# ZHKKKe/PixelSSL

Measured on NVIDIA H100. Metric: images/sec DeepLab-v2-R101 MT 513x513 bs16, higher is better.
Workload: dtype f16x3 (fp16 pairs, fp32 accumulate)

## Files before the change

### pixelssl_b200/csrc/conv_tc.cu

```cuda
#include "common.cuh"
#include <cuda.h>
#include <cstdlib>

typedef CUresult (*EncodeTiledFn)(CUtensorMap*, CUtensorMapDataType, cuuint32_t, void*, const cuuint64_t*,
                                  const cuuint64_t*, const cuuint32_t*, const cuuint32_t*, CUtensorMapInterleave,
                                  CUtensorMapSwizzle, CUtensorMapL2promotion, CUtensorMapFloatOOBfill);
static EncodeTiledFn get_encode() {
    static EncodeTiledFn fn = nullptr;
    if (!fn) {
        void* p = nullptr;
        cudaDriverEntryPointQueryResult q;
        if (cudaGetDriverEntryPoint("cuTensorMapEncodeTiled", &p, cudaEnableDefault, &q) == cudaSuccess &&
            q == cudaDriverEntryPointSuccess)
            fn = (EncodeTiledFn)p;
    }
    return fn;
}

static int make_act_map(CUtensorMap* m, const void* base, int C, int W, int H, int N, int bw, int bh, int estride = 1, int f16 = 0) {
    EncodeTiledFn enc = get_encode();
    if (!enc) return PXL_ERR_UNSUPPORTED;
    const cuuint64_t eb = f16 ? 2 : 4;
    cuuint64_t dims[4] = {(cuuint64_t)C, (cuuint64_t)W, (cuuint64_t)H, (cuuint64_t)N};
    cuuint64_t strides[3] = {(cuuint64_t)C * eb, (cuuint64_t)W * C * eb, (cuuint64_t)H * W * C * eb};
    cuuint32_t box[4] = {(cuuint32_t)(f16 ? 64 : 32), (cuuint32_t)(bw * estride), (cuuint32_t)(bh * estride), 1};
    cuuint32_t es[4] = {1, (cuuint32_t)estride, (cuuint32_t)estride, 1};
    if (box[1] > 256 || box[2] > 256) return PXL_ERR_UNSUPPORTED;
    CUresult r = enc(m, f16 ? CU_TENSOR_MAP_DATA_TYPE_FLOAT16 : CU_TENSOR_MAP_DATA_TYPE_FLOAT32, 4, (void*)base, dims, strides, box, es,
                     CU_TENSOR_MAP_INTERLEAVE_NONE, CU_TENSOR_MAP_SWIZZLE_128B, CU_TENSOR_MAP_L2_PROMOTION_L2_256B,
                     CU_TENSOR_MAP_FLOAT_OOB_FILL_NONE);
    return r == CUDA_SUCCESS ? 0 : PXL_ERR_BAD_ARG;
}

static int make_w_map(CUtensorMap* m, const void* base, int64_t K, int rows, int bn, int f16 = 0) {
    EncodeTiledFn enc = get_encode();
    if (!enc) return PXL_ERR_UNSUPPORTED;
    cuuint64_t dims[2] = {(cuuint64_t)K, (cuuint64_t)rows};
    cuuint64_t strides[1] = {(cuuint64_t)K * (f16 ? 2 : 4)};
    cuuint32_t box[2] = {(cuuint32_t)(f16 ? 64 : 32), (cuuint32_t)bn};
    cuuint32_t es[2] = {1, 1};
    CUresult r = enc(m, f16 ? CU_TENSOR_MAP_DATA_TYPE_FLOAT16 : CU_TENSOR_MAP_DATA_TYPE_FLOAT32, 2, (void*)base, dims, strides, box, es,
                     CU_TENSOR_MAP_INTERLEAVE_NONE, CU_TENSOR_MAP_SWIZZLE_128B, CU_TENSOR_MAP_L2_PROMOTION_L2_256B,
                     CU_TENSOR_MAP_FLOAT_OOB_FILL_NONE);
    return r == CUDA_SUCCESS ? 0 : PXL_ERR_BAD_ARG;
}

__device__ __forceinline__ uint32_t smem_u32(const void* p) { return (uint32_t)__cvta_generic_to_shared(p); }

__device__ __forceinline__ void mbar_init(uint64_t* bar, uint32_t count) {
    asm volatile("mbarrier.init.shared::cta.b64 [%0], %1;" ::"r"(smem_u32(bar)), "r"(count));
}
__device__ __forceinline__ void mbar_expect_tx(uint64_t* bar, uint32_t bytes) {
    asm volatile("mbarrier.arrive.expect_tx.shared::cta.b64 _, [%0], %1;" ::"r"(smem_u32(bar)), "r"(bytes) : "memory");
}
__device__ __forceinline__ void mbar_arrive(uint64_t* bar) {
    asm volatile("mbarrier.arrive.shared::cta.b64 _, [%0];" ::"r"(smem_u32(bar)) : "memory");
}
__device__ __forceinline__ bool mbar_try_wait(uint64_t* bar, uint32_t parity) {
    uint32_t ok;
    asm volatile(
        "{\n\t.reg .pred p;\n\t"
        "mbarrier.try_wait.parity.shared::cta.b64 p, [%1], %2;\n\t"
        "selp.u32 %0, 1, 0, p;\n\t}"
        : "=r"(ok)
        : "r"(smem_u32(bar)), "r"(parity)
        : "memory");
    return ok != 0;
}
__device__ __forceinline__ bool mbar_wait(uint64_t* bar, uint32_t parity, int* flag, int code) {
    for (uint32_t spin = 0; spin < (1u << 22); ++spin) {
        if (mbar_try_wait(bar, parity)) return true;
        if ((spin & 1023u) == 1023u && *(volatile int*)flag != 0) return false;
    }
    atomicCAS(flag, 0, code);
    return false;
}
__device__ __forceinline__ void tma_load_4d(void* dst, const CUtensorMap* map, uint64_t* bar, int c0, int c1, int c2, int c3) {
    asm volatile(
        "cp.async.bulk.tensor.4d.shared::cluster.global.mbarrier::complete_tx::bytes [%0], [%1, {%3, %4, %5, %6}], [%2];"
        ::"r"(smem_u32(dst)), "l"(map), "r"(smem_u32(bar)), "r"(c0), "r"(c1), "r"(c2), "r"(c3)
        : "memory");
}
__device__ __forceinline__ void tma_load_2d(void* dst, const CUtensorMap* map, uint64_t* bar, int c0, int c1) {
    asm volatile(
        "cp.async.bulk.tensor.2d.shared::cluster.global.mbarrier::complete_tx::bytes [%0], [%1, {%3, %4}], [%2];"
        ::"r"(smem_u32(dst)), "l"(map), "r"(smem_u32(bar)), "r"(c0), "r"(c1)
        : "memory");
}
__device__ __forceinline__ bool elect_one() {
    uint32_t pred = 0;
    asm volatile(
        "{\n\t.reg .b32 rx;\n\t.reg .pred px;\n\t"
        "elect.sync rx|px, 0xffffffff;\n\t"
        "@px mov.s32 %0, 1;\n\t}"
        : "+r"(pred));
    return pred != 0;
}
__device__ __forceinline__ void named_bar(int id, int count) {
    asm volatile("bar.sync %0, %1;" ::"r"(id), "r"(count) : "memory");
}
__device__ __forceinline__ void fence_async_smem() { asm volatile("fence.proxy.async.shared::cta;" ::: "memory"); }

__device__ __forceinline__ uint64_t sw128_desc(uint32_t smem_addr, uint32_t lbo_bytes = 16) {
    uint64_t d = 0;
    d |= (uint64_t)((smem_addr & 0x3FFFF) >> 4);
    d |= (uint64_t)((lbo_bytes >> 4) & 0x3FFF) << 16;
    d |= (uint64_t)(1024 >> 4) << 32;
    d |= (uint64_t)1 << 62;
    return d;
}
__device__ __forceinline__ void wg_arrive() { asm volatile("wgmma.fence.sync.aligned;" ::: "memory"); }
__device__ __forceinline__ void wg_commit() { asm volatile("wgmma.commit_group.sync.aligned;" ::: "memory"); }
__device__ __forceinline__ void wg_wait0() { asm volatile("wgmma.wait_group.sync.aligned 0;" ::: "memory"); }
template <int R>
__device__ __forceinline__ void fence_regs(float (&d)[R]) {
#pragma unroll
    for (int i = 0; i < R; ++i) asm volatile("" : "+f"(d[i])::"memory");
}

template <int N, int KIND>
__device__ __forceinline__ void wgmma_op(float (&d)[N / 2], uint64_t da, uint64_t db, int scale_d);
template <> __device__ __forceinline__ void wgmma_op<32, 0>(float (&d)[16], uint64_t da, uint64_t db, int scale_d) {
    asm volatile(
        "{\n\t.reg .pred p;\n\tsetp.ne.b32 p, %18, 0;\n\t"
        "wgmma.mma_async.sync.aligned.m64n32k8.f32.tf32.tf32 {%0, %1, %2, %3, %4, %5, %6, %7, %8, %9, %10, %11, %12, %13, %14, %15}, %16, %17, p, 1, 1;\n\t}"
        : "+f"(d[0]), "+f"(d[1]), "+f"(d[2]), "+f"(d[3]), "+f"(d[4]), "+f"(d[5]), "+f"(d[6]), "+f"(d[7]), "+f"(d[8]), "+f"(d[9]), "+f"(d[10]), "+f"(d[11]), "+f"(d[12]), "+f"(d[13]), "+f"(d[14]), "+f"(d[15])
        : "l"(da), "l"(db), "r"(scale_d));
}
template <> __device__ __forceinline__ void wgmma_op<64, 0>(float (&d)[32], uint64_t da, uint64_t db, int scale_d) {
    asm volatile(
        "{\n\t.reg .pred p;\n\tsetp.ne.b32 p, %34, 0;\n\t"
        "wgmma.mma_async.sync.aligned.m64n64k8.f32.tf32.tf32 {%0, %1, %2, %3, %4, %5, %6, %7, %8, %9, %10, %11, %12, %13, %14, %15, %16, %17, %18, %19, %20, %21, %22, %23, %24, %25, %26, %27, %28, %29, %30, %31}, %32, %33, p, 1, 1;\n\t}"
        : "+f"(d[0]), "+f"(d[1]), "+f"(d[2]), "+f"(d[3]), "+f"(d[4]), "+f"(d[5]), "+f"(d[6]), "+f"(d[7]), "+f"(d[8]), "+f"(d[9]), "+f"(d[10]), "+f"(d[11]), "+f"(d[12]), "+f"(d[13]), "+f"(d[14]), "+f"(d[15]), "+f"(d[16]), "+f"(d[17]), "+f"(d[18]), "+f"(d[19]), "+f"(d[20]), "+f"(d[21]), "+f"(d[22]), "+f"(d[23]), "+f"(d[24]), "+f"(d[25]), "+f"(d[26]), "+f"(d[27]), "+f"(d[28]), "+f"(d[29]), "+f"(d[30]), "+f"(d[31])
        : "l"(da), "l"(db), "r"(scale_d));
}
template <> __device__ __forceinline__ void wgmma_op<128, 0>(float (&d)[64], uint64_t da, uint64_t db, int scale_d) {
    asm volatile(
        "{\n\t.reg .pred p;\n\tsetp.ne.b32 p, %66, 0;\n\t"
        "wgmma.mma_async.sync.aligned.m64n128k8.f32.tf32.tf32 {%0, %1, %2, %3, %4, %5, %6, %7, %8, %9, %10, %11, %12, %13, %14, %15, %16, %17, %18, %19, %20, %21, %22, %23, %24, %25, %26, %27, %28, %29, %30, %31, %32, %33, %34, %35, %36, %37, %38, %39, %40, %41, %42, %43, %44, %45, %46, %47, %48, %49, %50, %51, %52, %53, %54, %55, %56, %57, %58, %59, %60, %61, %62, %63}, %64, %65, p, 1, 1;\n\t}"
        : "+f"(d[0]), "+f"(d[1]), "+f"(d[2]), "+f"(d[3]), "+f"(d[4]), "+f"(d[5]), "+f"(d[6]), "+f"(d[7]), "+f"(d[8]), "+f"(d[9]), "+f"(d[10]), "+f"(d[11]), "+f"(d[12]), "+f"(d[13]), "+f"(d[14]), "+f"(d[15]), "+f"(d[16]), "+f"(d[17]), "+f"(d[18]), "+f"(d[19]), "+f"(d[20]), "+f"(d[21]), "+f"(d[22]), "+f"(d[23]), "+f"(d[24]), "+f"(d[25]), "+f"(d[26]), "+f"(d[27]), "+f"(d[28]), "+f"(d[29]), "+f"(d[30]), "+f"(d[31]), "+f"(d[32]), "+f"(d[33]), "+f"(d[34]), "+f"(d[35]), "+f"(d[36]), "+f"(d[37]), "+f"(d[38]), "+f"(d[39]), "+f"(d[40]), "+f"(d[41]), "+f"(d[42]), "+f"(d[43]), "+f"(d[44]), "+f"(d[45]), "+f"(d[46]), "+f"(d[47]), "+f"(d[48]), "+f"(d[49]), "+f"(d[50]), "+f"(d[51]), "+f"(d[52]), "+f"(d[53]), "+f"(d[54]), "+f"(d[55]), "+f"(d[56]), "+f"(d[57]), "+f"(d[58]), "+f"(d[59]), "+f"(d[60]), "+f"(d[61]), "+f"(d[62]), "+f"(d[63])
        : "l"(da), "l"(db), "r"(scale_d));
}
template <> __device__ __forceinline__ void wgmma_op<32, 1>(float (&d)[16], uint64_t da, uint64_t db, int scale_d) {
    asm volatile(
        "{\n\t.reg .pred p;\n\tsetp.ne.b32 p, %18, 0;\n\t"
        "wgmma.mma_async.sync.aligned.m64n32k16.f32.f16.f16 {%0, %1, %2, %3, %4, %5, %6, %7, %8, %9, %10, %11, %12, %13, %14, %15}, %16, %17, p, 1, 1, 0, 0;\n\t}"
        : "+f"(d[0]), "+f"(d[1]), "+f"(d[2]), "+f"(d[3]), "+f"(d[4]), "+f"(d[5]), "+f"(d[6]), "+f"(d[7]), "+f"(d[8]), "+f"(d[9]), "+f"(d[10]), "+f"(d[11]), "+f"(d[12]), "+f"(d[13]), "+f"(d[14]), "+f"(d[15])
        : "l"(da), "l"(db), "r"(scale_d));
}
template <> __device__ __forceinline__ void wgmma_op<64, 1>(float (&d)[32], uint64_t da, uint64_t db, int scale_d) {
    asm volatile(
        "{\n\t.reg .pred p;\n\tsetp.ne.b32 p, %34, 0;\n\t"
        "wgmma.mma_async.sync.aligned.m64n64k16.f32.f16.f16 {%0, %1, %2, %3, %4, %5, %6, %7, %8, %9, %10, %11, %12, %13, %14, %15, %16, %17, %18, %19, %20, %21, %22, %23, %24, %25, %26, %27, %28, %29, %30, %31}, %32, %33, p, 1, 1, 0, 0;\n\t}"
        : "+f"(d[0]), "+f"(d[1]), "+f"(d[2]), "+f"(d[3]), "+f"(d[4]), "+f"(d[5]), "+f"(d[6]), "+f"(d[7]), "+f"(d[8]), "+f"(d[9]), "+f"(d[10]), "+f"(d[11]), "+f"(d[12]), "+f"(d[13]), "+f"(d[14]), "+f"(d[15]), "+f"(d[16]), "+f"(d[17]), "+f"(d[18]), "+f"(d[19]), "+f"(d[20]), "+f"(d[21]), "+f"(d[22]), "+f"(d[23]), "+f"(d[24]), "+f"(d[25]), "+f"(d[26]), "+f"(d[27]), "+f"(d[28]), "+f"(d[29]), "+f"(d[30]), "+f"(d[31])
        : "l"(da), "l"(db), "r"(scale_d));
}
template <> __device__ __forceinline__ void wgmma_op<128, 1>(float (&d)[64], uint64_t da, uint64_t db, int scale_d) {
    asm volatile(
        "{\n\t.reg .pred p;\n\tsetp.ne.b32 p, %66, 0;\n\t"
        "wgmma.mma_async.sync.aligned.m64n128k16.f32.f16.f16 {%0, %1, %2, %3, %4, %5, %6, %7, %8, %9, %10, %11, %12, %13, %14, %15, %16, %17, %18, %19, %20, %21, %22, %23, %24, %25, %26, %27, %28, %29, %30, %31, %32, %33, %34, %35, %36, %37, %38, %39, %40, %41, %42, %43, %44, %45, %46, %47, %48, %49, %50, %51, %52, %53, %54, %55, %56, %57, %58, %59, %60, %61, %62, %63}, %64, %65, p, 1, 1, 0, 0;\n\t}"
        : "+f"(d[0]), "+f"(d[1]), "+f"(d[2]), "+f"(d[3]), "+f"(d[4]), "+f"(d[5]), "+f"(d[6]), "+f"(d[7]), "+f"(d[8]), "+f"(d[9]), "+f"(d[10]), "+f"(d[11]), "+f"(d[12]), "+f"(d[13]), "+f"(d[14]), "+f"(d[15]), "+f"(d[16]), "+f"(d[17]), "+f"(d[18]), "+f"(d[19]), "+f"(d[20]), "+f"(d[21]), "+f"(d[22]), "+f"(d[23]), "+f"(d[24]), "+f"(d[25]), "+f"(d[26]), "+f"(d[27]), "+f"(d[28]), "+f"(d[29]), "+f"(d[30]), "+f"(d[31]), "+f"(d[32]), "+f"(d[33]), "+f"(d[34]), "+f"(d[35]), "+f"(d[36]), "+f"(d[37]), "+f"(d[38]), "+f"(d[39]), "+f"(d[40]), "+f"(d[41]), "+f"(d[42]), "+f"(d[43]), "+f"(d[44]), "+f"(d[45]), "+f"(d[46]), "+f"(d[47]), "+f"(d[48]), "+f"(d[49]), "+f"(d[50]), "+f"(d[51]), "+f"(d[52]), "+f"(d[53]), "+f"(d[54]), "+f"(d[55]), "+f"(d[56]), "+f"(d[57]), "+f"(d[58]), "+f"(d[59]), "+f"(d[60]), "+f"(d[61]), "+f"(d[62]), "+f"(d[63])
        : "l"(da), "l"(db), "r"(scale_d));
}
template <> __device__ __forceinline__ void wgmma_op<64, 2>(float (&d)[32], uint64_t da, uint64_t db, int scale_d) {
    asm volatile(
        "{\n\t.reg .pred p;\n\tsetp.ne.b32 p, %34, 0;\n\t"
        "wgmma.mma_async.sync.aligned.m64n64k16.f32.f16.f16 {%0, %1, %2, %3, %4, %5, %6, %7, %8, %9, %10, %11, %12, %13, %14, %15, %16, %17, %18, %19, %20, %21, %22, %23, %24, %25, %26, %27, %28, %29, %30, %31}, %32, %33, p, 1, 1, 1, 1;\n\t}"
        : "+f"(d[0]), "+f"(d[1]), "+f"(d[2]), "+f"(d[3]), "+f"(d[4]), "+f"(d[5]), "+f"(d[6]), "+f"(d[7]), "+f"(d[8]), "+f"(d[9]), "+f"(d[10]), "+f"(d[11]), "+f"(d[12]), "+f"(d[13]), "+f"(d[14]), "+f"(d[15]), "+f"(d[16]), "+f"(d[17]), "+f"(d[18]), "+f"(d[19]), "+f"(d[20]), "+f"(d[21]), "+f"(d[22]), "+f"(d[23]), "+f"(d[24]), "+f"(d[25]), "+f"(d[26]), "+f"(d[27]), "+f"(d[28]), "+f"(d[29]), "+f"(d[30]), "+f"(d[31])
        : "l"(da), "l"(db), "r"(scale_d));
}
template <> __device__ __forceinline__ void wgmma_op<128, 2>(float (&d)[64], uint64_t da, uint64_t db, int scale_d) {
    asm volatile(
        "{\n\t.reg .pred p;\n\tsetp.ne.b32 p, %66, 0;\n\t"
        "wgmma.mma_async.sync.aligned.m64n128k16.f32.f16.f16 {%0, %1, %2, %3, %4, %5, %6, %7, %8, %9, %10, %11, %12, %13, %14, %15, %16, %17, %18, %19, %20, %21, %22, %23, %24, %25, %26, %27, %28, %29, %30, %31, %32, %33, %34, %35, %36, %37, %38, %39, %40, %41, %42, %43, %44, %45, %46, %47, %48, %49, %50, %51, %52, %53, %54, %55, %56, %57, %58, %59, %60, %61, %62, %63}, %64, %65, p, 1, 1, 1, 1;\n\t}"
        : "+f"(d[0]), "+f"(d[1]), "+f"(d[2]), "+f"(d[3]), "+f"(d[4]), "+f"(d[5]), "+f"(d[6]), "+f"(d[7]), "+f"(d[8]), "+f"(d[9]), "+f"(d[10]), "+f"(d[11]), "+f"(d[12]), "+f"(d[13]), "+f"(d[14]), "+f"(d[15]), "+f"(d[16]), "+f"(d[17]), "+f"(d[18]), "+f"(d[19]), "+f"(d[20]), "+f"(d[21]), "+f"(d[22]), "+f"(d[23]), "+f"(d[24]), "+f"(d[25]), "+f"(d[26]), "+f"(d[27]), "+f"(d[28]), "+f"(d[29]), "+f"(d[30]), "+f"(d[31]), "+f"(d[32]), "+f"(d[33]), "+f"(d[34]), "+f"(d[35]), "+f"(d[36]), "+f"(d[37]), "+f"(d[38]), "+f"(d[39]), "+f"(d[40]), "+f"(d[41]), "+f"(d[42]), "+f"(d[43]), "+f"(d[44]), "+f"(d[45]), "+f"(d[46]), "+f"(d[47]), "+f"(d[48]), "+f"(d[49]), "+f"(d[50]), "+f"(d[51]), "+f"(d[52]), "+f"(d[53]), "+f"(d[54]), "+f"(d[55]), "+f"(d[56]), "+f"(d[57]), "+f"(d[58]), "+f"(d[59]), "+f"(d[60]), "+f"(d[61]), "+f"(d[62]), "+f"(d[63])
        : "l"(da), "l"(db), "r"(scale_d));
}

template <int BN, int F16>
__device__ __forceinline__ void mma_slice(float (&part)[BN / 2], float (&corr)[BN / 2], uint64_t da, uint64_t db, uint64_t dal,
                                          uint64_t dbl, bool split3) {
#pragma unroll
    for (int k = 0; k < 4; ++k) wgmma_op<BN, F16>(part, da + 2 * k, db + 2 * k, k);
    if (split3) {
#pragma unroll
        for (int k = 0; k < 4; ++k) wgmma_op<BN, F16>(corr, dal + 2 * k, db + 2 * k, k);
#pragma unroll
        for (int k = 0; k < 4; ++k) wgmma_op<BN, F16>(corr, da + 2 * k, dbl + 2 * k, 1);
    }
}

__device__ __forceinline__ float4 tf32_split4(float4 v, float4& lo) {
    float4 h;
    const float* vp = &v.x; float* hp = &h.x; float* lp = &lo.x;
#pragma unroll
    for (int e = 0; e < 4; ++e) {
        uint32_t u;
        asm("cvt.rna.tf32.f32 %0, %1;" : "=r"(u) : "f"(vp[e]));
        u &= 0xFFFFE000u;
        hp[e] = __uint_as_float(u);
        lp[e] = vp[e] - hp[e];
    }
    return h;
}

struct TcParams {
    int Cin, Cout, ldo, ntaps, kchunks;
    int N, OH, OW;
    int BW, BH, tilesW, tilesH;
    int stages, nsplit;
    int a_inkernel;
    int in_mul;
    int out_mul, out_offy, out_offx, outH, outW;
    int ntilesN, pix_tiles, total_tiles;
    int kc;
    float out_scale;
    int out_acc;
    short dy[PXL_MAX_TAPS], dx[PXL_MAX_TAPS], widx[PXL_MAX_TAPS];
};

#define TC_A_BYTES (128 * 128)
#define TC_MAX_STAGES 8
#define TC_THREADS 384

__device__ __forceinline__ void tc_tile_coords(const TcParams& p, int tile, int bn, int& n0, int& w0, int& h0, int& n) {
    const int nt = tile / p.pix_tiles, pix = tile - nt * p.pix_tiles;
    const int tw = pix % p.tilesW, th = (pix / p.tilesW) % p.tilesH;
    n = pix / (p.tilesW * p.tilesH);
    w0 = tw * p.BW; h0 = th * p.BH; n0 = nt * bn;
}

template <int BN, int F16>
__global__ void __launch_bounds__(TC_THREADS, 1)
conv_wg_kernel(const __grid_constant__ CUtensorMap mapA, const __grid_constant__ CUtensorMap mapAlo,
               const __grid_constant__ CUtensorMap mapB, const __grid_constant__ CUtensorMap mapBlo,
               const TcParams p, const float* __restrict__ bias, float* __restrict__ out,
               double* __restrict__ stats, int* __restrict__ err_flag, const float* __restrict__ oscale_ptr) {
    extern __shared__ __align__(1024) uint8_t smem_raw[];
    __shared__ uint64_t full_bar[TC_MAX_STAGES], empty_bar[TC_MAX_STAGES];
    __shared__ float st_warp[2][8][BN];

    uint8_t* smem = (uint8_t*)(((uintptr_t)smem_raw + 1023) & ~(uintptr_t)1023);
    constexpr int B_BYTES = BN * 128;
    constexpr int PER_OP = TC_A_BYTES + B_BYTES;
    const int stage_bytes = PER_OP * (p.nsplit == 3 ? 2 : 1);
    const int iters = p.ntaps * p.kchunks;

    if (threadIdx.x == 0) {
        for (int s = 0; s < p.stages; ++s) { mbar_init(&full_bar[s], 1); mbar_init(&empty_bar[s], 256); }
        asm volatile("fence.mbarrier_init.release.cluster;" ::: "memory");
    }
    __syncthreads();
    PXL_PDL_SYNC();

    if (threadIdx.x < 128) {
        asm volatile("setmaxnreg.dec.sync.aligned.u32 40;" ::: "memory");
        if (threadIdx.x >= 32) return;
        uint32_t tx = (uint32_t)((p.BW * p.BH * 128 + B_BYTES) * (p.nsplit == 3 ? 2 : 1));
        if (p.a_inkernel) tx -= (uint32_t)(p.BW * p.BH * 128);
        uint32_t s = 0, ph = 0;
        bool ok = true;
        for (int tile = blockIdx.x; tile < p.total_tiles && ok; tile += gridDim.x) {
            int n0, w0, h0, n;
            tc_tile_coords(p, tile, BN, n0, w0, h0, n);
            int tap = 0, c0 = 0;
            for (int it = 0; it < iters; ++it) {
                ok = __all_sync(0xffffffffu, mbar_wait(&empty_bar[s], ph ^ 1u, err_flag, 1));
                if (!ok) break;
                uint8_t* sa = smem + (size_t)s * stage_bytes;
                const int ax = w0 * p.in_mul + p.dx[tap], ay = h0 * p.in_mul + p.dy[tap];
                const int bk = p.widx[tap] * p.Cin + c0;
                if (elect_one()) {
                    mbar_expect_tx(&full_bar[s], tx);
                    tma_load_4d(sa, &mapA, &full_bar[s], c0, ax, ay, n);
                    tma_load_2d(sa + TC_A_BYTES, &mapB, &full_bar[s], bk, n0);
                    if (p.nsplit == 3) {
                        if (!p.a_inkernel) tma_load_4d(sa + PER_OP, &mapAlo, &full_bar[s], c0, ax, ay, n);
                        tma_load_2d(sa + PER_OP + TC_A_BYTES, &mapBlo, &full_bar[s], bk, n0);
                    }
                }
                __syncwarp();
                c0 += p.kc; if (c0 >= p.Cin) { c0 = 0; ++tap; }
                if (++s == (uint32_t)p.stages) { s = 0; ph ^= 1u; }
            }
        }
        return;
    }

    asm volatile("setmaxnreg.inc.sync.aligned.u32 232;" ::: "memory");
    const int ct = threadIdx.x - 128;
    const int cw = ct >> 7, t = ct & 127;
    const int warp = t >> 5, lane = t & 31;
    const float osc = p.out_scale * (oscale_ptr ? __ldg(oscale_ptr) : 1.f);
    const uint32_t smem_base = smem_u32(smem);
    const bool split3 = p.nsplit == 3;
    float acc[BN / 2], part[BN / 2], corr[BN / 2];
    uint32_t s = 0, ph = 0;
    int st_n0 = -1;
    float st_s = 0.f, st_q = 0.f;
    bool ok = true;
    auto flush_stats = [&]() {
        if (st_n0 >= 0 && ct < BN && st_n0 + ct < p.Cout && (st_s != 0.f || st_q != 0.f)) {
            atomicAdd(stats + st_n0 + ct, (double)st_s);
            atomicAdd(stats + p.Cout + st_n0 + ct, (double)st_q);
        }
        st_s = 0.f; st_q = 0.f;
    };
    for (int tile = blockIdx.x; tile < p.total_tiles && ok; tile += gridDim.x) {
        int n0, w0, h0, n;
        tc_tile_coords(p, tile, BN, n0, w0, h0, n);
        if (stats && n0 != st_n0) { flush_stats(); st_n0 = n0; }
#pragma unroll
        for (int i = 0; i < BN / 2; ++i) acc[i] = 0.f;
        for (int it = 0; it < iters; ++it) {
            ok = __all_sync(0xffffffffu, mbar_wait(&full_bar[s], ph, err_flag, 2));
            if (!ok) break;
            uint8_t* sa = smem + (size_t)s * stage_bytes;
            if (p.a_inkernel) {
                float4* a_hi = reinterpret_cast<float4*>(sa + cw * (TC_A_BYTES / 2));
                float4* a_lo = reinterpret_cast<float4*>(sa + PER_OP + cw * (TC_A_BYTES / 2));
#pragma unroll
                for (int c = 0; c < TC_A_BYTES / 2 / 16 / 128; ++c) {
                    float4 lo;
                    const float4 hi = tf32_split4(a_hi[t + c * 128], lo);
                    a_hi[t + c * 128] = hi;
                    a_lo[t + c * 128] = lo;
                }
                fence_async_smem();
                named_bar(2 + cw, 128);
            }
            const uint32_t sa32 = smem_base + s * (uint32_t)stage_bytes;
            const uint32_t arow = (uint32_t)cw * (TC_A_BYTES / 2);
            const uint64_t da = sw128_desc(sa32 + arow), db = sw128_desc(sa32 + TC_A_BYTES);
            const uint64_t dal = sw128_desc(sa32 + PER_OP + arow), dbl = sw128_desc(sa32 + PER_OP + TC_A_BYTES);
            wg_arrive();
            fence_regs(part);
            fence_regs(corr);
#pragma unroll
            for (int k = 0; k < 2; ++k) wgmma_op<BN, F16>(part, da + 2 * k, db + 2 * k, k);
            if (split3) {
#pragma unroll
                for (int k = 0; k < 4; ++k) wgmma_op<BN, F16>(corr, dal + 2 * k, db + 2 * k, k);
#pragma unroll
                for (int k = 0; k < 4; ++k) wgmma_op<BN, F16>(corr, da + 2 * k, dbl + 2 * k, 1);
            }
            wg_commit();
            wg_wait0();
            fence_regs(part);
#pragma unroll
            for (int i = 0; i < BN / 2; ++i) acc[i] += part[i];
            wg_arrive();
            fence_regs(part);
#pragma unroll
            for (int k = 2; k < 4; ++k) wgmma_op<BN, F16>(part, da + 2 * k, db + 2 * k, k - 2);
            wg_commit();
            wg_wait0();
            fence_regs(part);
            fence_regs(corr);
            mbar_arrive(&empty_bar[s]);
            if (split3) {
#pragma unroll
                for (int i = 0; i < BN / 2; ++i) acc[i] += part[i] + corr[i];
            } else {
#pragma unroll
                for (int i = 0; i < BN / 2; ++i) acc[i] += part[i];
            }
            if (++s == (uint32_t)p.stages) { s = 0; ph ^= 1u; }
        }
        if (!ok) break;
        int64_t obase[2];
        bool valid[2];
#pragma unroll
        for (int h = 0; h < 2; ++h) {
            const int r = cw * 64 + warp * 16 + (lane >> 2) + 8 * h;
            const int hy = r / p.BW, wx = r - hy * p.BW;
            const int oy = h0 + hy, ox = w0 + wx;
            valid[h] = hy < p.BH && oy < p.OH && ox < p.OW;
            obase[h] = ((int64_t)(n * p.outH + oy * p.out_mul + p.out_offy) * p.outW + ox * p.out_mul + p.out_offx) * p.ldo;
        }
        const bool vec2 = (p.ldo & 1) == 0 && ((uintptr_t)out & 7) == 0;
#pragma unroll
        for (int j = 0; j < BN / 8; ++j) {
            const int cl = j * 8 + 2 * (lane & 3);
            const int col = n0 + cl;
            const bool c0ok = col < p.Cout, c1ok = col + 1 < p.Cout;
            const float b0 = (bias && c0ok) ? __ldg(bias + col) : 0.f, b1 = (bias && c1ok) ? __ldg(bias + col + 1) : 0.f;
            float v[2][2];
#pragma unroll
            for (int h = 0; h < 2; ++h) {
                v[h][0] = acc[j * 4 + 2 * h] * osc + b0;
                v[h][1] = acc[j * 4 + 2 * h + 1] * osc + b1;
                if (!valid[h]) continue;
                float* o = out + obase[h] + col;
                if (p.out_acc) {
                    if (c0ok) o[0] += v[h][0];
                    if (c1ok) o[1] += v[h][1];
                } else if (c1ok && vec2) {
                    *reinterpret_cast<float2*>(o) = make_float2(v[h][0], v[h][1]);
                } else {
                    if (c0ok) o[0] = v[h][0];
                    if (c1ok) o[1] = v[h][1];
                }
            }
            if (stats) {
                float s0 = (valid[0] ? v[0][0] : 0.f) + (valid[1] ? v[1][0] : 0.f);
                float s1 = (valid[0] ? v[0][1] : 0.f) + (valid[1] ? v[1][1] : 0.f);
                float q0 = (valid[0] ? v[0][0] * v[0][0] : 0.f) + (valid[1] ? v[1][0] * v[1][0] : 0.f);
                float q1 = (valid[0] ? v[0][1] * v[0][1] : 0.f) + (valid[1] ? v[1][1] * v[1][1] : 0.f);
#pragma unroll
                for (int o = 4; o < 32; o <<= 1) {
                    s0 += __shfl_xor_sync(0xffffffffu, s0, o); s1 += __shfl_xor_sync(0xffffffffu, s1, o);
                    q0 += __shfl_xor_sync(0xffffffffu, q0, o); q1 += __shfl_xor_sync(0xffffffffu, q1, o);
                }
                if (lane < 4) {
                    const int slot = cw * 4 + warp;
                    st_warp[0][slot][cl] = s0; st_warp[0][slot][cl + 1] = s1;
                    st_warp[1][slot][cl] = q0; st_warp[1][slot][cl + 1] = q1;
                }
            }
        }
        if (stats) {
            named_bar(1, 256);
            if (ct < BN) {
#pragma unroll
                for (int w8 = 0; w8 < 8; ++w8) { st_s += st_warp[0][w8][ct]; st_q += st_warp[1][w8][ct]; }
            }
            named_bar(1, 256);
        }
    }
    if (stats && ok) flush_stats();
}

__global__ void __launch_bounds__(256)
split_tf32_kernel(const float4* __restrict__ x, float4* __restrict__ hi, float4* __restrict__ lo, int64_t n4) {
    const int64_t stride = (int64_t)gridDim.x * blockDim.x;
    for (int64_t i = (int64_t)blockIdx.x * blockDim.x + threadIdx.x; i < n4; i += stride) {
        float4 l;
        hi[i] = tf32_split4(__ldcs(x + i), l);
        lo[i] = l;
    }
}

extern "C" int pxl_split_tf32(const float* x, float* hi, float* lo, int64_t n, void* stream) {
    if (!x || !hi || !lo || n <= 0 || (n & 3)) return PXL_ERR_BAD_ARG;
    const int64_t n4 = n / 4;
    int blocks = (int)(pxl_cdiv(n4, 256 * 2) < PXL_NUM_SMS * 8 ? pxl_cdiv(n4, 256 * 2) : PXL_NUM_SMS * 8);
    split_tf32_kernel<<<blocks, 256, 0, (cudaStream_t)stream>>>((const float4*)x, (float4*)hi, (float4*)lo, n4);
    PXL_CHECK_LAUNCH();
    return 0;
}

static int* g_err_flag = nullptr;

static int ensure_err_flag() {
    if (g_err_flag) return 0;
    cudaError_t e = cudaMalloc(&g_err_flag, sizeof(int));
    if (e != cudaSuccess) return (int)e;
    e = cudaMemset(g_err_flag, 0, sizeof(int));
    return e == cudaSuccess ? 0 : (int)e;
}

template <typename K>
static int query_dyn_smem_limit(K kernel) {
    int dev = 0, optin = 0;
    cudaFuncAttributes a;
    if (cudaGetDevice(&dev) != cudaSuccess || cudaDeviceGetAttribute(&optin, cudaDevAttrMaxSharedMemoryPerBlockOptin, dev) != cudaSuccess ||
        cudaFuncGetAttributes(&a, kernel) != cudaSuccess)
// ... 113 lines not shown
    p.ntilesN = (g->Cout + BN - 1) / BN;
    const int64_t n_tiles = (int64_t)p.pix_tiles * p.ntilesN;
    if (n_tiles >= (1ll << 31)) return PXL_ERR_UNSUPPORTED;
    p.total_tiles = (int)n_tiles;
    const int smem_limit = f16 ? (BN == 128 ? fwd_smem_limit<128, 1>() : BN == 64 ? fwd_smem_limit<64, 1>() : fwd_smem_limit<32, 1>())
                               : (BN == 128 ? fwd_smem_limit<128, 0>() : BN == 64 ? fwd_smem_limit<64, 0>() : fwd_smem_limit<32, 0>());
    if (smem_limit <= 0) return PXL_ERR_UNSUPPORTED;
    p.stages = (smem_limit - 1024) / stage_bytes;
    if (p.stages > TC_MAX_STAGES) p.stages = TC_MAX_STAGES;
    if (p.stages < 2) return PXL_ERR_UNSUPPORTED;
    const size_t smem = (size_t)p.stages * stage_bytes + 1024;

    CUtensorMap mA, mAlo, mB, mBlo;
    int rc = make_act_map(&mA, in_hi, g->Cin, mapW, mapH, mapN, p.BW, p.BH, g->mul, f16);
    if (rc) return rc;
    rc = make_w_map(&mB, w_hi, (int64_t)wtaps * g->Cin, g->Cout, BN, f16);
    if (rc) return rc;
    if (nsplit == 3) {
        if (a_inkernel) mAlo = mA;
        else {
            rc = make_act_map(&mAlo, in_lo, g->Cin, mapW, mapH, mapN, p.BW, p.BH, g->mul, f16);
            if (rc) return rc;
        }
        rc = make_w_map(&mBlo, w_lo, (int64_t)wtaps * g->Cin, g->Cout, BN, f16);
        if (rc) return rc;
    } else {
        mAlo = mA; mBlo = mB;
    }
    p.out_acc = (ext && ext->out_accumulate) ? 1 : 0;
    if ((rc = ensure_err_flag())) return rc;
    cudaStream_t st = (cudaStream_t)stream;
    double* st_ptr = ext ? (double*)ext->bn_stats : nullptr;
    if (f16) {
        if (BN == 128) return launch_fwd<128, 1>(mA, mAlo, mB, mBlo, p, smem, st, bias, out, st_ptr, oscale_ptr);
        if (BN == 64) return launch_fwd<64, 1>(mA, mAlo, mB, mBlo, p, smem, st, bias, out, st_ptr, oscale_ptr);
        return launch_fwd<32, 1>(mA, mAlo, mB, mBlo, p, smem, st, bias, out, st_ptr, oscale_ptr);
    }
    if (BN == 128) return launch_fwd<128, 0>(mA, mAlo, mB, mBlo, p, smem, st, bias, out, st_ptr, oscale_ptr);
    if (BN == 64) return launch_fwd<64, 0>(mA, mAlo, mB, mBlo, p, smem, st, bias, out, st_ptr, oscale_ptr);
    return launch_fwd<32, 0>(mA, mAlo, mB, mBlo, p, smem, st, bias, out, st_ptr, oscale_ptr);
}

extern "C" int pxl_conv_tc_status(void) {
    if (!g_err_flag) return 0;
    int v = 0;
    if (cudaMemcpy(&v, g_err_flag, sizeof(int), cudaMemcpyDeviceToHost) != cudaSuccess) return -1;
    return v;
}

extern "C" int pxl_conv_tc_impl(const pxl_conv_geom* g, const int* taps, const float* in, const float* w,
                                const float* bias, float* out, void* stream) {
    if (!g) return PXL_ERR_BAD_ARG;
    if (g->precision == 2) return PXL_ERR_UNSUPPORTED;
    return pxl_conv_tc_launch(g, taps, in, nullptr, w, nullptr, bias, out, stream);
}

struct WgParams {
    int Cin, Cout, ldo, ntaps;
    int N, OH, OW, mul;
    int BW, BH, tilesW, tilesH, rows, rows_alloc;
    int stages, nsplit;
    int inkernel;
    int slab_ch;
    float out_scale;
    int tiles_ci, ktiles_per_cta, ktiles_total;
    short dy[PXL_MAX_TAPS], dx[PXL_MAX_TAPS];
};

template <int BN, int F16>
__global__ void __launch_bounds__(TC_THREADS, 1)
conv_wgrad_wg_kernel(const __grid_constant__ CUtensorMap mapDy, const __grid_constant__ CUtensorMap mapDyLo,
                     const __grid_constant__ CUtensorMap mapX, const __grid_constant__ CUtensorMap mapXLo,
                     const WgParams p, float* __restrict__ dw, float* __restrict__ ws, int* __restrict__ err_flag,
                     const float* __restrict__ oscale_ptr) {
    extern __shared__ __align__(1024) uint8_t smem_raw[];
    __shared__ uint64_t full_bar[TC_MAX_STAGES], empty_bar[TC_MAX_STAGES];
    uint8_t* smem = (uint8_t*)(((uintptr_t)smem_raw + 1023) & ~(uintptr_t)1023);

    const int slab_bytes = p.rows_alloc * 128;
    const int slabsA = 128 / p.slab_ch;
    const int slabsB = BN / p.slab_ch;
    const int per_op = (slabsA + slabsB) * slab_bytes;
    const int stage_bytes = per_op * (p.nsplit == 3 ? 2 : 1);
    constexpr int KT_BYTES = (128 + BN) * 128;
    uint8_t* kt = smem + (size_t)p.stages * stage_bytes;
    const int tile_co = blockIdx.x / p.tiles_ci, tile_ci = blockIdx.x % p.tiles_ci;
    const int co0 = tile_co * 128, ci0 = tile_ci * BN;
    const int tap = blockIdx.y;
    const int kt0 = blockIdx.z * p.ktiles_per_cta;
    int kt1 = kt0 + p.ktiles_per_cta;
    if (kt1 > p.ktiles_total) kt1 = p.ktiles_total;
    const int iters = kt1 - kt0;
    int nsA = (p.ldo - co0 + p.slab_ch - 1) / p.slab_ch; if (nsA > slabsA) nsA = slabsA;
    int nsB = (p.Cin - ci0 + p.slab_ch - 1) / p.slab_ch; if (nsB > slabsB) nsB = slabsB;

    {
        uint4 z = make_uint4(0, 0, 0, 0);
        const int total16 = p.stages * stage_bytes / 16;
        for (int i = threadIdx.x; i < total16; i += blockDim.x) reinterpret_cast<uint4*>(smem)[i] = z;
        fence_async_smem();
    }
    if (threadIdx.x == 0) {
        for (int s = 0; s < p.stages; ++s) { mbar_init(&full_bar[s], 1); mbar_init(&empty_bar[s], 256); }
        asm volatile("fence.mbarrier_init.release.cluster;" ::: "memory");
    }
    __syncthreads();
    PXL_PDL_SYNC();
    if (iters <= 0) return;

    if (threadIdx.x < 128) {
        asm volatile("setmaxnreg.dec.sync.aligned.u32 40;" ::: "memory");
        if (threadIdx.x >= 32) return;
        const uint32_t box_bytes = (uint32_t)(p.rows * 128);
        const int nparts = (p.nsplit == 3 && !p.inkernel) ? 2 : 1;
        const uint32_t tx = box_bytes * (uint32_t)(nsA + nsB) * (uint32_t)nparts;
        const int tdy = p.dy[tap], tdx = p.dx[tap];
        int tw = kt0 % p.tilesW, th = (kt0 / p.tilesW) % p.tilesH, n = kt0 / (p.tilesW * p.tilesH);
        uint32_t s = 0, ph = 0;
        for (int it = 0; it < iters; ++it) {
            if (!__all_sync(0xffffffffu, mbar_wait(&empty_bar[s], ph ^ 1u, err_flag, 11))) break;
            const int w0 = tw * p.BW, h0 = th * p.BH;
            uint8_t* sa = smem + (size_t)s * stage_bytes;
            if (elect_one()) {
                mbar_expect_tx(&full_bar[s], tx);
                for (int part = 0; part < nparts; ++part) {
                    uint8_t* base = sa + (size_t)part * per_op;
                    const CUtensorMap* mdy = part ? &mapDyLo : &mapDy;
                    const CUtensorMap* mx = part ? &mapXLo : &mapX;
                    for (int j = 0; j < nsA; ++j)
                        tma_load_4d(base + (size_t)j * slab_bytes, mdy, &full_bar[s], co0 + p.slab_ch * j, w0, h0, n);
                    for (int j = 0; j < nsB; ++j)
                        tma_load_4d(base + (size_t)(slabsA + j) * slab_bytes, mx, &full_bar[s], ci0 + p.slab_ch * j,
                                    w0 * p.mul + tdx, h0 * p.mul + tdy, n);
                }
            }
            __syncwarp();
            if (++tw == p.tilesW) { tw = 0; if (++th == p.tilesH) { th = 0; ++n; } }
            if (++s == (uint32_t)p.stages) { s = 0; ph ^= 1u; }
        }
        return;
    }

    asm volatile("setmaxnreg.inc.sync.aligned.u32 232;" ::: "memory");
    const int ct = threadIdx.x - 128;
    const int cw = ct >> 7, t = ct & 127;
    const int warp = t >> 5, lane = t & 31;
    const bool split3 = p.nsplit == 3;
    const uint32_t smem_base = smem_u32(smem);
    float acc[BN / 2], part[BN / 2], corr[BN / 2];
#pragma unroll
    for (int i = 0; i < BN / 2; ++i) acc[i] = 0.f;
    uint32_t s = 0, ph = 0;
    bool ok = true;
    for (int it = 0; it < iters; ++it) {
        ok = __all_sync(0xffffffffu, mbar_wait(&full_bar[s], ph, err_flag, 12));
        if (!ok) break;
        uint8_t* sa = smem + (size_t)s * stage_bytes;
        const uint32_t sa32 = smem_base + s * (uint32_t)stage_bytes;
        if constexpr (F16 != 0) {
            const int kmma = p.rows_alloc / 16;
            const uint32_t sb32 = sa32 + (uint32_t)(slabsA * slab_bytes);
            const uint64_t da = sw128_desc(sa32 + (uint32_t)(cw * slab_bytes), (uint32_t)slab_bytes);
            const uint64_t db = sw128_desc(sb32, (uint32_t)slab_bytes);
            const uint64_t dal = sw128_desc(sa32 + (uint32_t)per_op + (uint32_t)(cw * slab_bytes), (uint32_t)slab_bytes);
            const uint64_t dbl = sw128_desc(sb32 + (uint32_t)per_op, (uint32_t)slab_bytes);
            const uint64_t kstep = (16 * 128) >> 4;
            wg_arrive();
            fence_regs(part);
            fence_regs(corr);
            for (int k = 0; k < kmma; ++k) wgmma_op<BN, 2>(part, da + kstep * k, db + kstep * k, k);
            if (split3) {
                for (int k = 0; k < kmma; ++k) wgmma_op<BN, 2>(corr, dal + kstep * k, db + kstep * k, k);
                for (int k = 0; k < kmma; ++k) wgmma_op<BN, 2>(corr, da + kstep * k, dbl + kstep * k, 1);
            }
            wg_commit();
            wg_wait0();
            fence_regs(part);
            fence_regs(corr);
            mbar_arrive(&empty_bar[s]);
        } else {
            named_bar(1, 256);
            const int units = (128 + BN) * 8;
            for (int u = ct; u < units; u += 256) {
                const int R = u >> 3, g = u & 7;
                const int slab = R < 128 ? (R >> 5) : slabsA + ((R - 128) >> 5);
                const int c = R & 31;
                const uint8_t* src = sa + (size_t)slab * slab_bytes + (c & 3) * 4;
                float4 v, vl = make_float4(0.f, 0.f, 0.f, 0.f);
                float* vp = &v.x; float* lp = &vl.x;
#pragma unroll
                for (int e = 0; e < 4; ++e) {
                    const int px = 4 * g + e;
                    const int off = px * 128 + ((((c >> 2) ^ (px & 7))) << 4);
                    vp[e] = *reinterpret_cast<const float*>(src + off);
                    if (split3 && !p.inkernel) lp[e] = *reinterpret_cast<const float*>(src + per_op + off);
                }
                if (p.inkernel) v = tf32_split4(v, vl);
                const int doff = R * 128 + ((g ^ (R & 7)) << 4);
                *reinterpret_cast<float4*>(kt + doff) = v;
                if (split3) *reinterpret_cast<float4*>(kt + KT_BYTES + doff) = vl;
            }
            fence_async_smem();
            named_bar(1, 256);
            mbar_arrive(&empty_bar[s]);
            const uint32_t k32 = smem_u32(kt);
            const uint32_t arow = (uint32_t)cw * 64 * 128;
            const uint64_t da = sw128_desc(k32 + arow), db = sw128_desc(k32 + 128 * 128);
            const uint64_t dal = sw128_desc(k32 + KT_BYTES + arow), dbl = sw128_desc(k32 + KT_BYTES + 128 * 128);
            wg_arrive();
            fence_regs(part);
            fence_regs(corr);
            mma_slice<BN, 0>(part, corr, da, db, dal, dbl, split3);
            wg_commit();
            wg_wait0();
            fence_regs(part);
            fence_regs(corr);
        }
        if (split3) {
#pragma unroll
            for (int i = 0; i < BN / 2; ++i) acc[i] += part[i] + corr[i];
        } else {
#pragma unroll
            for (int i = 0; i < BN / 2; ++i) acc[i] += part[i];
        }
        if (++s == (uint32_t)p.stages) { s = 0; ph ^= 1u; }
    }
    if (!ok) return;
    const float osc = p.out_scale * (oscale_ptr ? __ldg(oscale_ptr) : 1.f);
#pragma unroll
    for (int h = 0; h < 2; ++h) {
        const int co = co0 + cw * 64 + warp * 16 + (lane >> 2) + 8 * h;
        if (co >= p.Cout) continue;
        const int64_t row = ((int64_t)co * p.ntaps + tap) * p.Cin;
        float* drow = gridDim.z == 1 ? dw + row : ws + (int64_t)blockIdx.z * p.Cout * p.ntaps * p.Cin + row;
#pragma unroll
        for (int j = 0; j < BN / 8; ++j) {
            const int ci = ci0 + j * 8 + 2 * (lane & 3);
            const float v0 = acc[j * 4 + 2 * h] * osc, v1 = acc[j * 4 + 2 * h + 1] * osc;
            if (gridDim.z == 1) {
                if (ci < p.Cin) drow[ci] += v0;
                if (ci + 1 < p.Cin) drow[ci + 1] += v1;
            } else {
                if (ci < p.Cin) drow[ci] = v0;
                if (ci + 1 < p.Cin) drow[ci + 1] = v1;
            }
        }
    }
}

__global__ void __launch_bounds__(256)
wgrad_reduce_kernel(const float* __restrict__ ws, float* __restrict__ dw, int64_t n, int splits) {
    const int64_t stride = (int64_t)gridDim.x * blockDim.x;
    for (int64_t i = (int64_t)blockIdx.x * blockDim.x + threadIdx.x; i < n; i += stride) {
        float s = __ldg(ws + i);
        for (int z = 1; z < splits; ++z) s += __ldg(ws + (int64_t)z * n + i);
        dw[i] += s;
    }
}

static int make_act_map_strided(CUtensorMap* m, const void* base, int C, int W, int H, int N, int bw, int bh, int estride, int f16 = 0) {
    return make_act_map(m, base, C, W, H, N, bw, bh, estride, f16);
}

static void pick_ktile(int OH, int OW, bool flat, int maxrows, int& BW, int& BH, int unit = 8) {
    if (flat) { BW = maxrows; BH = 1; return; }
    double best = -1.0;
    BW = 8; BH = maxrows / 8;
    for (int bw = 1; bw <= maxrows && bw <= 256; ++bw) {
        int bh = maxrows / bw;
        if (bh < 1) break;
        if (bh > 256) bh = 256;
        const int alloc = (bw * bh + unit - 1) / unit * unit;
        const int64_t tiles = (int64_t)((OW + bw - 1) / bw) * ((OH + bh - 1) / bh);
        const double eff = (double)OH * OW / ((double)tiles * alloc);
        if (eff > best + 1e-9) { best = eff; BW = bw; BH = bh; }
    }
}

static int conv_wgrad_tc_core(const pxl_conv_geom* g, const int* taps, const void* in_hi, const void* in_lo,
                              const void* dy_hi, const void* dy_lo, float* dw, float out_scale, const float* oscale_ptr,
                              void* stream);

extern "C" int pxl_conv_wgrad_tc_launch(const pxl_conv_geom* g, const int* taps, const float* in_hi, const float* in_lo,
                                        const float* dy_hi, const float* dy_lo, float* dw, void* stream) {
    if (g && g->precision > 2) return PXL_ERR_BAD_ARG;
    return conv_wgrad_tc_core(g, taps, in_hi, in_lo, dy_hi, dy_lo, dw, 1.f, nullptr, stream);
}

extern "C" int pxl_conv_wgrad_h16_launch(const pxl_conv_geom* g, const int* taps, const void* in_hi, const void* in_lo,
                                         const void* dy_hi, const void* dy_lo, float* dw, float out_scale,
                                         const float* out_scale_dev, void* stream) {
    if (!g || (g->precision != 3 && g->precision != 4)) return PXL_ERR_BAD_ARG;
    return conv_wgrad_tc_core(g, taps, in_hi, in_lo, dy_hi, dy_lo, dw, out_scale != 0.f ? out_scale : 1.f, out_scale_dev, stream);
}

template <int BN, int F16>
static int wgrad_smem_limit() {
    static const int v = query_dyn_smem_limit(conv_wgrad_wg_kernel<BN, F16>);
    return v;
}

template <int BN, int F16>
static int launch_wgrad(const CUtensorMap& mDy, const CUtensorMap& mDyLo, const CUtensorMap& mX, const CUtensorMap& mXLo,
                        const WgParams& p, dim3 grid, size_t smem, cudaStream_t st, float* dw, const float* oscale_ptr) {
    static bool attr = false;
    if (!attr) {
        cudaError_t e = cudaFuncSetAttribute(conv_wgrad_wg_kernel<BN, F16>, cudaFuncAttributeMaxDynamicSharedMemorySize, wgrad_smem_limit<BN, F16>());
        if (e != cudaSuccess) return (int)e;
        attr = true;
    }
    const int64_t n = (int64_t)p.Cout * p.ntaps * p.Cin;
    float* ws = nullptr;
    if (grid.z > 1) {
        int rc = 0;
        ws = (float*)pxl_workspace_(PXL_WS_WGRAD, st, (size_t)n * grid.z * sizeof(float), &rc);
        if (rc) return rc;
    }
    cudaError_t le = pxl_launch_pdl(conv_wgrad_wg_kernel<BN, F16>, grid, dim3(TC_THREADS), smem, st, mDy, mDyLo, mX, mXLo, p, dw,
                                    ws, g_err_flag, oscale_ptr);
    if (le != cudaSuccess) return (int)le;
    PXL_CHECK_LAUNCH();
    if (grid.z > 1) {
        const int blocks = (int)(pxl_cdiv(n, 256) < PXL_NUM_SMS * 8 ? pxl_cdiv(n, 256) : PXL_NUM_SMS * 8);
        wgrad_reduce_kernel<<<blocks, 256, 0, st>>>(ws, dw, n, (int)grid.z);
        PXL_CHECK_LAUNCH();
    }
    return 0;
}

static int conv_wgrad_tc_core(const pxl_conv_geom* g, const int* taps, const void* in_hi, const void* in_lo,
                              const void* dy_hi, const void* dy_lo, float* dw, float out_scale, const float* oscale_ptr,
                              void* stream) {
    if (!g || !taps || !in_hi || !dy_hi || !dw) return PXL_ERR_BAD_ARG;
    if (g->div != 1 || (g->mul != 1 && g->mul != 2)) return PXL_ERR_UNSUPPORTED;
    const int f16 = g->precision >= 3 ? 1 : 0;
    const int slab_ch = f16 ? 64 : 32;
    if (g->Cin % slab_ch != 0 || g->ldo % slab_ch != 0 || g->ntaps > PXL_MAX_TAPS) return PXL_ERR_UNSUPPORTED;
    const int nsplit = (g->precision == 2 || g->precision == 3) ? 3 : 1;
    if (nsplit == 3 && ((in_lo == nullptr) != (dy_lo == nullptr))) return PXL_ERR_BAD_ARG;
    if (f16 && nsplit == 3 && !in_lo) return PXL_ERR_BAD_ARG;
    const int inkernel = (!f16 && nsplit == 3 && !in_lo) ? 1 : 0;
    const bool flat = (g->ntaps == 1 && taps[0] == 0 && taps[1] == 0 && g->OH == g->H && g->OW == g->W && g->mul == 1);
    WgParams p;
    p.Cin = g->Cin; p.Cout = g->Cout; p.ldo = g->ldo; p.ntaps = g->ntaps; p.mul = g->mul; p.nsplit = nsplit; p.inkernel = inkernel;
    p.slab_ch = slab_ch; p.out_scale = out_scale;
    for (int t = 0; t < g->ntaps; ++t) { p.dy[t] = (short)taps[2 * t]; p.dx[t] = (short)taps[2 * t + 1]; }
    int mapW, mapH, mapN, inW, inH;
    if (flat) {
        const int64_t M = (int64_t)g->N * g->H * g->W;
        if (M >= (1ll << 31)) return PXL_ERR_UNSUPPORTED;
        p.N = 1; p.OH = 1; p.OW = (int)M; mapW = (int)M; mapH = 1; mapN = 1; inW = (int)M; inH = 1;
    } else {
        p.N = g->N; p.OH = g->OH; p.OW = g->OW; mapW = g->OW; mapH = g->OH; mapN = g->N; inW = g->W; inH = g->H;
    }
    const int maxrows = f16 ? (nsplit == 3 ? 64 : 128) : 32;
    const int kunit = f16 ? 16 : 8;
    pick_ktile(p.OH, p.OW, flat, maxrows, p.BW, p.BH, kunit);
    p.rows = p.BW * p.BH;
    p.rows_alloc = f16 ? (p.rows + kunit - 1) / kunit * kunit : 32;
    p.tilesW = (p.OW + p.BW - 1) / p.BW; p.tilesH = (p.OH + p.BH - 1) / p.BH;
    const int BN = f16 ? (g->Cin > 64 ? 128 : 64) : (g->Cin > 64 ? 128 : (g->Cin > 32 ? 64 : 32));
    p.tiles_ci = (g->Cin + BN - 1) / BN;
    const int tiles_co = (g->Cout + 127) / 128;
    const int stage_bytes = (128 / slab_ch + BN / slab_ch) * p.rows_alloc * 128 * (nsplit == 3 ? 2 : 1);
    const int kt_bytes = f16 ? 0 : (128 + BN) * 128 * (nsplit == 3 ? 2 : 1);
    const int smem_limit = f16 ? (BN == 128 ? wgrad_smem_limit<128, 1>() : wgrad_smem_limit<64, 1>())
                               : (BN == 128 ? wgrad_smem_limit<128, 0>() : BN == 64 ? wgrad_smem_limit<64, 0>() : wgrad_smem_limit<32, 0>());
    if (smem_limit <= 0) return PXL_ERR_UNSUPPORTED;
    p.stages = (smem_limit - 1024 - kt_bytes) / stage_bytes;
    if (p.stages > 4) p.stages = 4;
// ... 49 lines not shown
```

Baseline: 160.3.

## Pipeline fp16 wgmma groups and specialize weight-grad loop on compile-time K

In the forward fp16 tensor-core path, the per-stage wgmma work is split into two commit groups so accumulation of one partial overlaps the next MMA group. In the non-split path, release of the smem stage is deferred by one iteration to keep MMAs in flight. The weight-gradient fp16 loop becomes a template on the MMA count and split3 flag, so the K loop fully unrolls and descriptor math is constant. This adds code size and more complex barrier ordering across stages.

```diff
diff --git a/pixelssl_b200/csrc/conv_tc.cu b/pixelssl_b200/csrc/conv_tc.cu
--- a/pixelssl_b200/csrc/conv_tc.cu
+++ b/pixelssl_b200/csrc/conv_tc.cu
@@ -1,6 +1,7 @@
 #include "common.cuh"
 #include <cuda.h>
 #include <cstdlib>
+#include <type_traits>
 
 typedef CUresult (*EncodeTiledFn)(CUtensorMap*, CUtensorMapDataType, cuuint32_t, void*, const cuuint64_t*,
                                   const cuuint64_t*, const cuuint32_t*, const cuuint32_t*, CUtensorMapInterleave,
@@ -306,13 +307,80 @@
         }
         st_s = 0.f; st_q = 0.f;
     };
+    auto f16_tile = [&](auto split3_c) -> bool {
+        constexpr bool S3 = decltype(split3_c)::value;
+        uint32_t prev = 0;
+        for (int it = 0; it < iters; ++it) {
+            if (!__all_sync(0xffffffffu, mbar_wait(&full_bar[s], ph, err_flag, 2))) { wg_wait0(); return false; }
+            const uint32_t sa32 = smem_base + s * (uint32_t)stage_bytes;
+            const uint32_t arow = (uint32_t)cw * (TC_A_BYTES / 2);
+            const uint64_t da = sw128_desc(sa32 + arow), db = sw128_desc(sa32 + TC_A_BYTES);
+            const uint64_t dal = sw128_desc(sa32 + PER_OP + arow), dbl = sw128_desc(sa32 + PER_OP + TC_A_BYTES);
+            wg_arrive();
+            fence_regs(part);
+            if (S3) fence_regs(corr);
+#pragma unroll
+            for (int k = 0; k < 2; ++k) wgmma_op<BN, 1>(part, da + 2 * k, db + 2 * k, k);
+            wg_commit();
+            if (S3) {
+#pragma unroll
+                for (int k = 0; k < 4; ++k) wgmma_op<BN, 1>(corr, dal + 2 * k, db + 2 * k, k);
+#pragma unroll
+                for (int k = 0; k < 4; ++k) wgmma_op<BN, 1>(corr, da + 2 * k, dbl + 2 * k, 1);
+                wg_commit();
+                asm volatile("wgmma.wait_group.sync.aligned 1;" ::: "memory");
+                fence_regs(part);
+#pragma unroll
+                for (int i = 0; i < BN / 2; ++i) acc[i] += part[i];
+                wg_arrive();
+                fence_regs(part);
+#pragma unroll
+                for (int k = 2; k < 4; ++k) wgmma_op<BN, 1>(part, da + 2 * k, db + 2 * k, k - 2);
+                wg_commit();
+                wg_wait0();
+                fence_regs(part);
+                fence_regs(corr);
+                mbar_arrive(&empty_bar[s]);
+#pragma unroll
+                for (int i = 0; i < BN / 2; ++i) acc[i] += part[i] + corr[i];
+            } else {
+                asm volatile("wgmma.wait_group.sync.aligned 1;" ::: "memory");
+                fence_regs(corr);
+                if (it > 0) {
+                    mbar_arrive(&empty_bar[prev]);
+#pragma unroll
+                    for (int i = 0; i < BN / 2; ++i) acc[i] += corr[i];
+                }
+                wg_arrive();
+                fence_regs(corr);
+#pragma unroll
+                for (int k = 2; k < 4; ++k) wgmma_op<BN, 1>(corr, da + 2 * k, db + 2 * k, k - 2);
+                wg_commit();
+                asm volatile("wgmma.wait_group.sync.aligned 1;" ::: "memory");
+                fence_regs(part);
+#pragma unroll
+                for (int i = 0; i < BN / 2; ++i) acc[i] += part[i];
+            }
+            prev = s;
+            if (++s == (uint32_t)p.stages) { s = 0; ph ^= 1u; }
+        }
+        if (!S3) {
+            wg_wait0();
+            fence_regs(corr);
+            mbar_arrive(&empty_bar[prev]);
+#pragma unroll
+            for (int i = 0; i < BN / 2; ++i) acc[i] += corr[i];
+        }
+        return true;
+    };
     for (int tile = blockIdx.x; tile < p.total_tiles && ok; tile += gridDim.x) {
         int n0, w0, h0, n;
         tc_tile_coords(p, tile, BN, n0, w0, h0, n);
         if (stats && n0 != st_n0) { flush_stats(); st_n0 = n0; }
 #pragma unroll
         for (int i = 0; i < BN / 2; ++i) acc[i] = 0.f;
-        for (int it = 0; it < iters; ++it) {
+        if constexpr (F16 != 0) ok = split3 ? f16_tile(std::true_type{}) : f16_tile(std::false_type{});
+        else for (int it = 0; it < iters; ++it) {
             ok = __all_sync(0xffffffffu, mbar_wait(&full_bar[s], ph, err_flag, 2));
             if (!ok) break;
             uint8_t* sa = smem + (size_t)s * stage_bytes;
@@ -732,70 +800,110 @@
     for (int i = 0; i < BN / 2; ++i) acc[i] = 0.f;
     uint32_t s = 0, ph = 0;
     bool ok = true;
-    for (int it = 0; it < iters; ++it) {
+    if constexpr (F16 != 0) {
+        auto f16_loop = [&](auto km_c, auto split3_c) -> bool {
+            constexpr int KM = decltype(km_c)::value;
+            constexpr bool S3 = decltype(split3_c)::value;
+            constexpr uint64_t kstep = (16 * 128) >> 4;
+            constexpr uint32_t SLAB = KM * 16 * 128;
+            constexpr uint32_t PER_OP = (128 + BN) / 64 * SLAB;
+            for (int it = 0; it < iters; ++it) {
+                if (!__all_sync(0xffffffffu, mbar_wait(&full_bar[s], ph, err_flag, 12))) return false;
+                const uint32_t sa32 = smem_base + s * (uint32_t)stage_bytes;
+                const uint32_t sb32 = sa32 + 2 * SLAB;
+                const uint64_t da = sw128_desc(sa32 + cw * SLAB, SLAB);
+                const uint64_t db = sw128_desc(sb32, SLAB);
+                wg_arrive();
+                fence_regs(part);
+                fence_regs(corr);
+#pragma unroll
+                for (int k = 0; k < KM; ++k) wgmma_op<BN, 2>(part, da + kstep * k, db + kstep * k, k);
+                if (S3) {
+                    const uint64_t dal = sw128_desc(sa32 + PER_OP + cw * SLAB, SLAB);
+                    const uint64_t dbl = sw128_desc(sb32 + PER_OP, SLAB);
+#pragma unroll
+                    for (int k = 0; k < KM; ++k) wgmma_op<BN, 2>(corr, dal + kstep * k, db + kstep * k, k);
+#pragma unroll
+                    for (int k = 0; k < KM; ++k) wgmma_op<BN, 2>(corr, da + kstep * k, dbl + kstep * k, 1);
+                }
+                wg_commit();
+                wg_wait0();
+                fence_regs(part);
+                fence_regs(corr);
+                mbar_arrive(&empty_bar[s]);
+                if (S3) {
+#pragma unroll
+                    for (int i = 0; i < BN / 2; ++i) acc[i] += part[i] + corr[i];
+                } else {
+#pragma unroll
+                    for (int i = 0; i < BN / 2; ++i) acc[i] += part[i];
+                }
+                if (++s == (uint32_t)p.stages) { s = 0; ph ^= 1u; }
+            }
+            return true;
+        };
+        using std::integral_constant;
+        using T = std::true_type;
+        using F = std::false_type;
+        if (split3) {
+            switch (p.rows_alloc / 16) {
+                case 1: ok = f16_loop(integral_constant<int, 1>{}, T{}); break;
+                case 2: ok = f16_loop(integral_constant<int, 2>{}, T{}); break;
+                case 3: ok = f16_loop(integral_constant<int, 3>{}, T{}); break;
+                default: ok = f16_loop(integral_constant<int, 4>{}, T{}); break;
+            }
+        } else {
+            switch (p.rows_alloc / 16) {
+                case 1: ok = f16_loop(integral_constant<int, 1>{}, F{}); break;
+                case 2: ok = f16_loop(integral_constant<int, 2>{}, F{}); break;
+                case 3: ok = f16_loop(integral_constant<int, 3>{}, F{}); break;
+                case 4: ok = f16_loop(integral_constant<int, 4>{}, F{}); break;
+                case 5: ok = f16_loop(integral_constant<int, 5>{}, F{}); break;
+                case 6: ok = f16_loop(integral_constant<int, 6>{}, F{}); break;
+                case 7: ok = f16_loop(integral_constant<int, 7>{}, F{}); break;
+                default: ok = f16_loop(integral_constant<int, 8>{}, F{}); break;
+            }
+        }
+    } else for (int it = 0; it < iters; ++it) {
         ok = __all_sync(0xffffffffu, mbar_wait(&full_bar[s], ph, err_flag, 12));
         if (!ok) break;
         uint8_t* sa = smem + (size_t)s * stage_bytes;
-        const uint32_t sa32 = smem_base + s * (uint32_t)stage_bytes;
-        if constexpr (F16 != 0) {
-            const int kmma = p.rows_alloc / 16;
-            const uint32_t sb32 = sa32 + (uint32_t)(slabsA * slab_bytes);
-            const uint64_t da = sw128_desc(sa32 + (uint32_t)(cw * slab_bytes), (uint32_t)slab_bytes);
-            const uint64_t db = sw128_desc(sb32, (uint32_t)slab_bytes);
-            const uint64_t dal = sw128_desc(sa32 + (uint32_t)per_op + (uint32_t)(cw * slab_bytes), (uint32_t)slab_bytes);
-            const uint64_t dbl = sw128_desc(sb32 + (uint32_t)per_op, (uint32_t)slab_bytes);
-            const uint64_t kstep = (16 * 128) >> 4;
-            wg_arrive();
-            fence_regs(part);
-            fence_regs(corr);
-            for (int k = 0; k < kmma; ++k) wgmma_op<BN, 2>(part, da + kstep * k, db + kstep * k, k);
-            if (split3) {
-                for (int k = 0; k < kmma; ++k) wgmma_op<BN, 2>(corr, dal + kstep * k, db + kstep * k, k);
-                for (int k = 0; k < kmma; ++k) wgmma_op<BN, 2>(corr, da + kstep * k, dbl + kstep * k, 1);
-            }
-            wg_commit();
-            wg_wait0();
-            fence_regs(part);
-            fence_regs(corr);
-            mbar_arrive(&empty_bar[s]);
-        } else {
-            named_bar(1, 256);
-            const int units = (128 + BN) * 8;
-            for (int u = ct; u < units; u += 256) {
-                const int R = u >> 3, g = u & 7;
-                const int slab = R < 128 ? (R >> 5) : slabsA + ((R - 128) >> 5);
-                const int c = R & 31;
-                const uint8_t* src = sa + (size_t)slab * slab_bytes + (c & 3) * 4;
-                float4 v, vl = make_float4(0.f, 0.f, 0.f, 0.f);
-                float* vp = &v.x; float* lp = &vl.x;
-#pragma unroll
-                for (int e = 0; e < 4; ++e) {
-                    const int px = 4 * g + e;
-                    const int off = px * 128 + ((((c >> 2) ^ (px & 7))) << 4);
-                    vp[e] = *reinterpret_cast<const float*>(src + off);
-                    if (split3 && !p.inkernel) lp[e] = *reinterpret_cast<const float*>(src + per_op + off);
-                }
-                if (p.inkernel) v = tf32_split4(v, vl);
-                const int doff = R * 128 + ((g ^ (R & 7)) << 4);
-                *reinterpret_cast<float4*>(kt + doff) = v;
-                if (split3) *reinterpret_cast<float4*>(kt + KT_BYTES + doff) = vl;
-            }
-            fence_async_smem();
-            named_bar(1, 256);
-            mbar_arrive(&empty_bar[s]);
-            const uint32_t k32 = smem_u32(kt);
-            const uint32_t arow = (uint32_t)cw * 64 * 128;
-            const uint64_t da = sw128_desc(k32 + arow), db = sw128_desc(k32 + 128 * 128);
-            const uint64_t dal = sw128_desc(k32 + KT_BYTES + arow), dbl = sw128_desc(k32 + KT_BYTES + 128 * 128);
-            wg_arrive();
-            fence_regs(part);
-            fence_regs(corr);
-            mma_slice<BN, 0>(part, corr, da, db, dal, dbl, split3);
-            wg_commit();
-            wg_wait0();
-            fence_regs(part);
-            fence_regs(corr);
-        }
+        named_bar(1, 256);
+        const int units = (128 + BN) * 8;
+        for (int u = ct; u < units; u += 256) {
+            const int R = u >> 3, g = u & 7;
+            const int slab = R < 128 ? (R >> 5) : slabsA + ((R - 128) >> 5);
+            const int c = R & 31;
+            const uint8_t* src = sa + (size_t)slab * slab_bytes + (c & 3) * 4;
+            float4 v, vl = make_float4(0.f, 0.f, 0.f, 0.f);
+            float* vp = &v.x; float* lp = &vl.x;
+#pragma unroll
+            for (int e = 0; e < 4; ++e) {
+                const int px = 4 * g + e;
+                const int off = px * 128 + ((((c >> 2) ^ (px & 7))) << 4);
+                vp[e] = *reinterpret_cast<const float*>(src + off);
+                if (split3 && !p.inkernel) lp[e] = *reinterpret_cast<const float*>(src + per_op + off);
+            }
+            if (p.inkernel) v = tf32_split4(v, vl);
+            const int doff = R * 128 + ((g ^ (R & 7)) << 4);
+            *reinterpret_cast<float4*>(kt + doff) = v;
+            if (split3) *reinterpret_cast<float4*>(kt + KT_BYTES + doff) = vl;
+        }
+        fence_async_smem();
+        named_bar(1, 256);
+        mbar_arrive(&empty_bar[s]);
+        const uint32_t k32 = smem_u32(kt);
+        const uint32_t arow = (uint32_t)cw * 64 * 128;
+        const uint64_t da = sw128_desc(k32 + arow), db = sw128_desc(k32 + 128 * 128);
+        const uint64_t dal = sw128_desc(k32 + KT_BYTES + arow), dbl = sw128_desc(k32 + KT_BYTES + 128 * 128);
+        wg_arrive();
+        fence_regs(part);
+        fence_regs(corr);
+        mma_slice<BN, 0>(part, corr, da, db, dal, dbl, split3);
+        wg_commit();
+        wg_wait0();
+        fence_regs(part);
+        fence_regs(corr);
         if (split3) {
 #pragma unroll
             for (int i = 0; i < BN / 2; ++i) acc[i] += part[i] + corr[i];
```

Measured after the change: 167.2, median of 6. 4.3% higher.
